# LiuZhu-CV/PAIF

Hardware: AMD Instinct MI355X
Metric: fused image-pairs/sec at 480x640 bs=8 per GPU (fusion-net forward) (higher is better)
Workload: dtype f16 (IEEE fp16 maps and conv weights, one fp16 MFMA per product, f32 accumulate; stems, guided filter and the last map fp32)

## Files before the change

paif_amd/csrc/conv_dma.hip:

```cpp
#include <stdint.h>
#include <stdlib.h>

#include <type_traits>

#include "conv_dma.h"
#include "paif_common.h"

namespace paif_conv_dma {
namespace {

typedef float f32x16 __attribute__((ext_vector_type(16)));
typedef unsigned u32x4 __attribute__((ext_vector_type(4)));
constexpr int TW = 32, TH = 8;
#ifndef CD_PF
#define CD_PF 4
#endif
#ifndef CD_ST_AUX
#define CD_ST_AUX 2
#endif
#ifndef CD_EXP
#define CD_EXP 0
#endif
constexpr int PARK_WAVE = 2 * 32 * 32 * 4;
template <int DIL>
struct Geo {
  static constexpr int TWH = TW + 2 * DIL, THH = TH + 2 * DIL;
  static constexpr int NPIX = TWH * THH;
  static constexpr int DPW = (NPIX * 4 + 255) / 256;
  static constexpr int SLOT = 4 * DPW * 1024;
  static constexpr int PF = DIL == 1 ? CD_PF : 3;
  static constexpr int NSLOT = PF + 1;
  static constexpr int ROWB = TWH * 64;
  static constexpr int PARK_OFF = NSLOT * SLOT;
  static constexpr int LDS_BYTES = PARK_OFF + 4 * PARK_WAVE;
  static_assert(LDS_BYTES <= 160 * 1024, "ring + transposition buffers exceed LDS");
  static_assert(4 * DPW * 64 >= NPIX * 4, "DMA instructions do not cover the halo tile");
  static __device__ __forceinline__ int base_row(int w) { return DIL == 1 ? 2 * w : (w >> 1) * 4 + (w & 1); }
};
constexpr unsigned RSRC_W3 = 0x00020000u;
constexpr unsigned OOB = 0x80000000u;
constexpr int NSTORE = 4;
constexpr int VMCAP = 63;

#define CD_VMWAIT(n) asm volatile("s_waitcnt vmcnt(%0)" ::"n"((n) > VMCAP ? VMCAP : (n)) : "memory")
#define CD_RD128(dst, addr, off) asm volatile("ds_read_b128 %0, %1 offset:%2" : "=v"(dst) : "v"(addr), "n"(off) : "memory")
#define CD_WR32(addr, val, off) asm volatile("ds_write_b32 %0, %1 offset:%2" ::"v"(addr), "v"(val), "n"(off) : "memory")

__device__ __forceinline__ void dma16(__amdgpu_buffer_rsrc_t rsrc, unsigned voff, unsigned lds_off) {
  __builtin_amdgcn_raw_ptr_buffer_load_lds(rsrc, (__attribute__((address_space(3))) void*)(uintptr_t)lds_off, 16, voff, 0, 0, 0);
}

template <int NSRC, int NRES, int PF, int DPW>
struct Sched {
  static constexpr int RL = 4 * NRES;
  static constexpr int smod(int x) { return ((x % NSRC) + NSRC) % NSRC; }
  static constexpr int R_STAGE = smod(1 - PF);
  static constexpr int D = (R_STAGE + PF - 1 - NSRC) / NSRC;
  static constexpr int U = D + (R_STAGE == 0 ? 2 : 1);
  static_assert(PF >= 2 && D >= 0 && U <= 4, "prefetch distance out of the range the tile loop lists");
  static constexpr int n1 = DPW * (PF - 1);
};

template <int NSRC, int NRES, int F, bool CP = false, int DIL = 1, int IA = 0>
__global__ __launch_bounds__(256, 1) void conv3x3_h16_dma(Args a, int ntiles, int tilesX, int tilesY) {
  typedef Geo<DIL> G;
  constexpr int TWH = G::TWH, NPIX = G::NPIX, DPW = G::DPW, SLOT = G::SLOT, PF = G::PF, NSLOT = G::NSLOT, ROWB = G::ROWB, PARK_OFF = G::PARK_OFF;
  typedef Sched<NSRC, NRES, PF, DPW> SC;
  constexpr int U = SC::U, D = SC::D;
  __shared__ __attribute__((aligned(16))) unsigned char smem[G::LDS_BYTES];
  asm volatile("" ::"v"((unsigned)(uintptr_t)(__attribute__((address_space(3))) unsigned char*)smem) : "memory");

  const int tid = threadIdx.x, l = tid & 63;
  const int w = __builtin_amdgcn_readfirstlane(tid >> 6);
  const int p = l & 31, hh = l >> 5;
  const int wb = G::base_row(w);

  const int xcd = blockIdx.x & 7, wg = blockIdx.x >> 3, nwg = gridDim.x >> 3;
  const int tpx = (ntiles + 7) >> 3;
  const int t_beg = xcd * tpx, t_end = min(ntiles, t_beg + tpx);
  const int cnt = t_beg + wg < t_end ? (t_end - t_beg - wg + nwg - 1) / nwg : 0;
  if (cnt == 0) return;
  const int H = a.H, W = a.W;
  auto pack_tile = [&](int k) -> unsigned {
    const int pos = wg + min(k, cnt - 1) * nwg;
    int t = a.reverse ? t_end - 1 - pos : t_beg + pos;
    const int tx = t % tilesX;
    t /= tilesX;
    const int ty = t % tilesY;
    return ((unsigned)(t / tilesY) << 22) | ((unsigned)ty << 11) | (unsigned)tx;
  };
  const unsigned tab0 = pack_tile(l), tab1 = pack_tile(l + 64);
  auto tile_of = [&](int k, int& b, int& y0, int& x0) -> bool {
    const bool ok = k >= 0 && k < cnt;
    const int kk = ok ? k : 0;
    const unsigned lo = __builtin_amdgcn_readlane(tab0, kk & 63), hi = __builtin_amdgcn_readlane(tab1, kk & 63);
    const unsigned pk = kk < 64 ? lo : hi;
    b = pk >> 22; y0 = ((pk >> 11) & 2047) * TH; x0 = (pk & 2047) * TW;
    return ok;
  };

  const int map_bytes = a.B * H * W * 64;
  __amdgpu_buffer_rsrc_t rs_src[NSRC];
#pragma unroll
  for (int s = 0; s < NSRC; ++s) rs_src[s] = __builtin_amdgcn_make_buffer_rsrc(const_cast<void*>(a.src[s]), 0, map_bytes, RSRC_W3);
  __amdgpu_buffer_rsrc_t rs_res[NRES > 0 ? NRES : 1];
#pragma unroll
  for (int r = 0; r < NRES; ++r) rs_res[r] = __builtin_amdgcn_make_buffer_rsrc(const_cast<void*>(a.res[r]), 0, map_bytes, RSRC_W3);
  const int opitch = a.cout * 2;
  const __amdgpu_buffer_rsrc_t rs_out = __builtin_amdgcn_make_buffer_rsrc(a.out, 0, a.B * H * W * opitch, RSRC_W3);
  const __amdgpu_buffer_rsrc_t rs_null = __builtin_amdgcn_make_buffer_rsrc(a.out, 0, 0, RSRC_W3);
  const __amdgpu_buffer_rsrc_t rs_cp = __builtin_amdgcn_make_buffer_rsrc(CP ? (void*)a.cpool : a.out, 0, CP ? a.B * H * W * 16 - 8 : 0, RSRC_W3);

  u32x4 bw[NSRC][9][2];
  {
    const __amdgpu_buffer_rsrc_t rs_w = __builtin_amdgcn_make_buffer_rsrc(const_cast<void*>(a.wpk), 0, NSRC * 9 * 2 * 2 * 1024, RSRC_W3);
#pragma unroll
    for (int s = 0; s < NSRC; ++s)
#pragma unroll
      for (int tap = 0; tap < 9; ++tap)
#pragma unroll
        for (int ks = 0; ks < 2; ++ks)
          bw[s][tap][ks] = __builtin_amdgcn_raw_buffer_load_b128(rs_w, (unsigned)l * 16u, (((s * 9 + tap) * 2 + ks) * 2) * 1024, 0);
  }
  float esc[8], esh[8];
#pragma unroll
  for (int j = 0; j < 8; ++j) {
    const int c = 8 * (l & 3) + j;
    esc[j] = ((a.scale && c < a.cout) ? a.scale[c] : 1.f) * a.alpha;
    esh[j] = ((a.shift && c < a.cout) ? a.shift[c] : 0.f) * a.alpha;
  }
  const float e_slope = a.act == 1 ? *a.prelu : (a.act == 2 ? 0.f : 1.f);

  int d_rel[DPW];
  int d_rc[DPW];
#pragma unroll
  for (int i = 0; i < DPW; ++i) {
    const int n = (w * DPW + i) * 64 + l;
    const int pi = n >> 2;
    const int r = pi / TWH, c = pi - r * TWH;
    d_rel[i] = (r * W + c) * 64 + (((n & 3) ^ ((c >> 2) & 3)) * 16);
    d_rc[i] = pi < NPIX ? (r | (c << 8)) : -1;
  }
  unsigned d_voff[DPW];
  auto target = [&](int k) {
    int b, y0, x0;
    const bool ok = tile_of(k, b, y0, x0);
    const int org = ((b * H + y0 - DIL) * W + x0 - DIL) * 64;
#pragma unroll
    for (int i = 0; i < DPW; ++i) {
      const int gy = y0 - DIL + (d_rc[i] & 0xff), gx = x0 - DIL + (d_rc[i] >> 8);
      const bool in = !(CD_EXP & 4) && ok && d_rc[i] >= 0 && (unsigned)gy < (unsigned)H && (unsigned)gx < (unsigned)W;
      d_voff[i] = in ? (unsigned)(org + d_rel[i]) : OOB;
    }
  };
  unsigned a_rd[3][2];
#pragma unroll
  for (int dx = 0; dx < 3; ++dx)
#pragma unroll
    for (int ks = 0; ks < 2; ++ks) {
      const int c = p + dx * DIL;
      a_rd[dx][ks] = (unsigned)(wb * ROWB + c * 64 + (((2 * ks + hh) ^ ((c >> 2) & 3)) * 16));
    }
  const unsigned a_pw = PARK_OFF + w * PARK_WAVE + (4 * hh * 32 + p) * 4;
  const unsigned a_pr = PARK_OFF + w * PARK_WAVE + (l >> 2) * 128 + (l & 3) * 32;
  const unsigned e_lane = (unsigned)l * 16u;
  const unsigned o_lane = 8 * (l & 3) < a.cout ? (unsigned)((l >> 2) * opitch + (l & 3) * 16) : OOB;

  u32x4 rr[U][NRES > 0 ? NRES : 1][4];
  auto issue_res = [&](auto settag, int k) {
    constexpr int SET = decltype(settag)::value;
    int b, y0, x0;
    const bool ok = tile_of(k, b, y0, x0);
#pragma unroll
    for (int it = 0; it < 4; ++it) {
      const int y = y0 + wb + (it >> 1) * DIL, x = x0 + (it & 1) * 16 + (l >> 2);
      const bool in = ok && y < H && x < W;
      const unsigned soff = (unsigned)(((b * H + y) * W + x0 + (it & 1) * 16) * 64);
#pragma unroll
      for (int r = 0; r < NRES; ++r) rr[SET][r][it] = __builtin_amdgcn_raw_buffer_load_b128(rs_res[r], in ? e_lane : OOB, soff, 0);
    }
  };

  auto relu_frag = [](u32x4& f) {
    typedef short s16x8 __attribute__((ext_vector_type(8)));
    const s16x8 z = {0, 0, 0, 0, 0, 0, 0, 0};
    f = __builtin_bit_cast(u32x4, __builtin_elementwise_max(__builtin_bit_cast(s16x8, f), z));
  };
  f32x16 acc[2];
  u32x4 t[4][2];
#pragma unroll
  for (int it = 0; it < 4; ++it) t[it][0] = t[it][1] = u32x4{0, 0, 0, 0};
  float ev[8];
  float pmx = 0.f, psm = 0.f;
  int cur = NSLOT - PF;

  auto epi = [&](auto mtag, auto settag, bool pok, int pb, int py0, int px0) {
    constexpr int M = decltype(mtag)::value, SETP = decltype(settag)::value;
    constexpr int it = M / 9, j = M % 9;
    if constexpr (j < 8) {
      const unsigned raw = j < 4 ? t[it][0][j & 3] : t[it][1][j & 3];
      float v = __builtin_fmaf(__uint_as_float(raw), esc[j], esh[j]);
      v = __builtin_fmaf(e_slope, fminf(v, 0.f), fmaxf(v, 0.f));
#pragma unroll
      for (int r = 0; r < NRES; ++r) {
        const unsigned u = rr[SETP][r][it][j >> 1];
        if constexpr (F == 2) v += (float)__builtin_bit_cast(paif::f16x2_t, u)[j & 1];
        else v += __uint_as_float((j & 1) ? (u & 0xffff0000u) : (u << 16));
      }
      ev[j] = v;
      if constexpr (CP) {
        pmx = j == 0 ? v : fmaxf(pmx, v);
        psm = j == 0 ? v : psm + v;
      }
    } else {
      const uint2 o0 = paif::f32_to_h4<F>(make_float4(ev[0], ev[1], ev[2], ev[3]));
      const uint2 o1 = paif::f32_to_h4<F>(make_float4(ev[4], ev[5], ev[6], ev[7]));
      const int y = py0 + wb + (it >> 1) * DIL, x = px0 + (it & 1) * 16 + (l >> 2);
      const unsigned soff = (unsigned)(((pb * H + y) * W + px0 + (it & 1) * 16) * opitch);
      u32x4 od = {o0.x, o0.y, o1.x, o1.y};
      __builtin_amdgcn_raw_buffer_store_b128(od, rs_out, (!(CD_EXP & 1) && pok && y < H && x < W) ? o_lane : OOB, soff, CD_ST_AUX);
      asm volatile("s_nop 2" : "+v"(od));
      if constexpr (CP) {
        float mx = pmx, sm = psm;
        mx = fmaxf(mx, paif::dpp_f<0xB1>(mx)); sm += paif::dpp_f<0xB1>(sm);
        mx = fmaxf(mx, paif::dpp_f<0x4E>(mx)); sm += paif::dpp_f<0x4E>(sm);
        typedef float f32x2v __attribute__((ext_vector_type(2)));
        const f32x2v pv = {mx, sm * (1.0f / 32.0f)};
        const unsigned poff = (unsigned)(((pb * H + y) * W + px0 + (it & 1) * 16) * 16);
        __builtin_amdgcn_raw_buffer_store_b64(__builtin_bit_cast(unsigned __attribute__((ext_vector_type(2))), pv), rs_cp,
                                              (pok && y < H && x < W && (l & 3) == 0) ? (unsigned)((l >> 2) * 16) : OOB, poff, 0);
      }
    }
  };

  auto stage = [&](auto ktag, auto stag, auto virt, int k) {
    constexpr int K = decltype(ktag)::value, S = decltype(stag)::value;
    constexpr bool VIRT = decltype(virt)::value;
    constexpr int SETP = (K + U - 1) % U;
    const unsigned sb = (unsigned)cur * SLOT;
    const int fill = cur == 0 ? NSLOT - 1 : cur - 1;
    u32x4 A[2][4];
    unsigned ad[3][2];
    if constexpr (!VIRT) {
      CD_VMWAIT(SC::n1);
      asm volatile("s_barrier" ::: "memory");
#pragma unroll
      for (int dx = 0; dx < 3; ++dx)
#pragma unroll
        for (int ks = 0; ks < 2; ++ks) ad[dx][ks] = a_rd[dx][ks] + sb;
      if constexpr (S == 0) {
#pragma unroll
        for (int it = 0; it < 4; ++it) {
          CD_RD128(t[it][0], a_pr, it * 2048);
          CD_RD128(t[it][1], a_pr, it * 2048 + 16);
        }
      }
#pragma unroll
      for (int r = 0; r < 4; ++r) CD_RD128(A[0][r], ad[0][0], r * DIL * ROWB);
    }
    if constexpr (NRES > 0 && S == SC::R_STAGE) issue_res(std::integral_constant<int, (K + D) % U>{}, k + D);
    asm volatile("" ::: "memory");
    if constexpr ((S + PF) % NSRC == 0) target(k + (S + PF) / NSRC);
#pragma unroll
    for (int i = 0; i < DPW; ++i) dma16(rs_src[(S + PF) % NSRC], d_voff[i], (unsigned)(fill * SLOT + (w * DPW + i) * 1024));
    if constexpr (VIRT) {
      if constexpr (S == 0) {
#pragma unroll
        for (int it = 0; it < NSTORE; ++it) __builtin_amdgcn_raw_buffer_store_b128(u32x4{0, 0, 0, 0}, rs_null, 0, 0, 0);
      }
    } else {
      int pb = 0, py0 = 0, px0 = 0;
      bool pok = false;
      if constexpr (S == 0) pok = tile_of(k - 1, pb, py0, px0);
      auto mma = [&](auto gitag, auto dytag, auto jtag) {
        constexpr int gi = decltype(gitag)::value, dy = decltype(dytag)::value, j = decltype(jtag)::value;
        constexpr int ks = gi / 3, dx = gi % 3;
        if constexpr (!((CD_EXP & 2) && (dy > 0 || j > 0))) {
          const u32x4 av = A[gi & 1][j + dy], bv = bw[S][dy * 3 + dx][ks];
          if constexpr (S == 0 && gi == 0 && dy == 0) {
            const f32x16 z = {0.f, 0.f, 0.f, 0.f, 0.f, 0.f, 0.f, 0.f, 0.f, 0.f, 0.f, 0.f, 0.f, 0.f, 0.f, 0.f};
            acc[j] = paif::mfma16<F>(av, bv, z);
          } else {
            acc[j] = paif::mfma16<F>(av, bv, acc[j]);
          }
        }
        if constexpr (S == 0) epi(std::integral_constant<int, gi * 6 + dy * 2 + j>{}, std::integral_constant<int, SETP>{}, pok, pb, py0, px0);
        if constexpr (IA == 2) {
          constexpr int call = dy * 2 + j;
          if constexpr (call == 0) relu_frag(A[gi & 1][1]);
          if constexpr (call == 2) relu_frag(A[gi & 1][2]);
          if constexpr (call == 4) relu_frag(A[gi & 1][3]);
        }
        __builtin_amdgcn_sched_barrier(0);
      };
      auto group = [&](auto gitag) {
        constexpr int gi = decltype(gitag)::value;
        if constexpr (gi + 1 < 6) {
          constexpr int ks1 = (gi + 1) / 3, dx1 = (gi + 1) % 3;
#pragma unroll
          for (int r = 0; r < 4; ++r) CD_RD128(A[(gi + 1) & 1][r], ad[dx1][ks1], r * DIL * ROWB);
        }
        if constexpr (S == 0 && gi == 0) {
          asm volatile("s_waitcnt lgkmcnt(4)"
                       : "+v"(A[0][0]), "+v"(A[0][1]), "+v"(A[0][2]), "+v"(A[0][3]), "+v"(t[0][0]), "+v"(t[0][1]), "+v"(t[1][0]), "+v"(t[1][1]),
                         "+v"(t[2][0]), "+v"(t[2][1]), "+v"(t[3][0]), "+v"(t[3][1])::"memory");
        } else if constexpr (gi + 1 < 6) {
          asm volatile("s_waitcnt lgkmcnt(4)" : "+v"(A[gi & 1][0]), "+v"(A[gi & 1][1]), "+v"(A[gi & 1][2]), "+v"(A[gi & 1][3])::"memory");
        } else {
          asm volatile("s_waitcnt lgkmcnt(0)" : "+v"(A[gi & 1][0]), "+v"(A[gi & 1][1]), "+v"(A[gi & 1][2]), "+v"(A[gi & 1][3])::"memory");
        }
        if constexpr (IA == 2) relu_frag(A[gi & 1][0]);
        __builtin_amdgcn_sched_barrier(0);
        typedef std::integral_constant<int, 0> I0;
        typedef std::integral_constant<int, 1> I1;
        typedef std::integral_constant<int, 2> I2;
        mma(gitag, I0{}, I0{}); mma(gitag, I0{}, I1{});
        mma(gitag, I1{}, I0{}); mma(gitag, I1{}, I1{});
        mma(gitag, I2{}, I0{}); mma(gitag, I2{}, I1{});
      };
      group(std::integral_constant<int, 0>{});
      group(std::integral_constant<int, 1>{});
      group(std::integral_constant<int, 2>{});
      group(std::integral_constant<int, 3>{});
      group(std::integral_constant<int, 4>{});
      group(std::integral_constant<int, 5>{});
      if constexpr (S == NSRC - 1) {
        asm volatile("s_nop 15\n\ts_nop 7" ::: "memory");
#pragma unroll
        for (int j = 0; j < 2; ++j)
#pragma unroll
          for (int r = 0; r < 16; ++r) {
            const float v = acc[j][r];
            CD_WR32(a_pw, v, (j * 32 + (r & 3) + 8 * (r >> 2)) * 128);
          }
      }
    }
    cur = cur == NSLOT - 1 ? 0 : cur + 1;
  };
  auto drain = [&](auto ktag, int k) {
    constexpr int K = decltype(ktag)::value;
#pragma unroll
    for (int it = 0; it < 4; ++it) {
      CD_RD128(t[it][0], a_pr, it * 2048);
      CD_RD128(t[it][1], a_pr, it * 2048 + 16);
    }
    asm volatile("s_waitcnt lgkmcnt(0)"
                 : "+v"(t[0][0]), "+v"(t[0][1]), "+v"(t[1][0]), "+v"(t[1][1]), "+v"(t[2][0]), "+v"(t[2][1]), "+v"(t[3][0]), "+v"(t[3][1])::"memory");
    int pb, py0, px0;
    const bool pok = tile_of(k, pb, py0, px0);
#define CD_M(m) epi(std::integral_constant<int, m>{}, std::integral_constant<int, K>{}, pok, pb, py0, px0);
    CD_M(0) CD_M(1) CD_M(2) CD_M(3) CD_M(4) CD_M(5) CD_M(6) CD_M(7) CD_M(8) CD_M(9) CD_M(10) CD_M(11)
    CD_M(12) CD_M(13) CD_M(14) CD_M(15) CD_M(16) CD_M(17) CD_M(18) CD_M(19) CD_M(20) CD_M(21) CD_M(22) CD_M(23)
    CD_M(24) CD_M(25) CD_M(26) CD_M(27) CD_M(28) CD_M(29) CD_M(30) CD_M(31) CD_M(32) CD_M(33) CD_M(34) CD_M(35)
#undef CD_M
  };

  auto vstage = [&](auto jtag) {
    constexpr int J = decltype(jtag)::value;
    constexpr int T = (J - (NSRC - 1)) / NSRC;
    constexpr int S = J - T * NSRC;
    constexpr int K = ((T % U) + U) % U;
    stage(std::integral_constant<int, K>{}, std::integral_constant<int, S>{}, std::true_type{}, T);
  };
  static_assert(PF >= 1 && PF <= 4, "the prologue lists up to 4 virtual stages");
  if constexpr (PF >= 4) vstage(std::integral_constant<int, -4>{});
  if constexpr (PF >= 3) vstage(std::integral_constant<int, -3>{});
  if constexpr (PF >= 2) vstage(std::integral_constant<int, -2>{});
  vstage(std::integral_constant<int, -1>{});

  auto tile_step = [&](auto ktag, int k) {
    stage(ktag, std::integral_constant<int, 0>{}, std::false_type{}, k);
    if constexpr (NSRC > 1) stage(ktag, std::integral_constant<int, 1>{}, std::false_type{}, k);
    if constexpr (NSRC > 2) stage(ktag, std::integral_constant<int, 2>{}, std::false_type{}, k);
  };
  for (int k = 0;; k += U) {
    tile_step(std::integral_constant<int, 0>{}, k);
    if (k + 1 >= cnt) { drain(std::integral_constant<int, 0>{}, k); break; }
    if constexpr (U > 1) {
      tile_step(std::integral_constant<int, 1 % U>{}, k + 1);
      if (k + 2 >= cnt) { drain(std::integral_constant<int, 1 % U>{}, k + 1); break; }
    }
    if constexpr (U > 2) {
      tile_step(std::integral_constant<int, 2 % U>{}, k + 2);
      if (k + 3 >= cnt) { drain(std::integral_constant<int, 2 % U>{}, k + 2); break; }
    }
    if constexpr (U > 3) {
      tile_step(std::integral_constant<int, 3 % U>{}, k + 3);
      if (k + 4 >= cnt) { drain(std::integral_constant<int, 3 % U>{}, k + 3); break; }
    }
  }
  CD_VMWAIT(0);
}

namespace k7 {
constexpr int P = 3;
constexpr int TWH = TW + 2 * P, THH = TH + 2 * P;
constexpr int NPIX = TWH * THH;
constexpr int DPW = 9;
constexpr int SLOT = 4 * DPW * 1024;
constexpr int NSLOT = 2;
constexpr int ROWB = TWH * 64;
constexpr int WB_OFF = NSLOT * SLOT;
constexpr int WB_BYTES = 49 * 1024;
constexpr int PARK_OFF = WB_OFF + WB_BYTES;
constexpr int LDS_BYTES = PARK_OFF + 4 * PARK_WAVE;
static_assert(LDS_BYTES <= 160 * 1024, "7x7: ring + weights + transposition buffers exceed LDS");
static_assert(4 * DPW * 64 >= NPIX * 4, "7x7: DMA instructions do not cover the halo tile");
}

#define CD_WR128(addr, val, off) asm volatile("ds_write_b128 %0, %1 offset:%2" ::"v"(addr), "v"(val), "n"(off) : "memory")

template <int F>
__global__ __launch_bounds__(256, 1) void conv7x7_h16_dma(Args a, int ntiles, int tilesX, int tilesY) {
  constexpr int P = k7::P, TWH = k7::TWH, NPIX = k7::NPIX, DPW = k7::DPW, SLOT = k7::SLOT, ROWB = k7::ROWB, WB_OFF = k7::WB_OFF,
                PARK_OFF = k7::PARK_OFF;
  __shared__ __attribute__((aligned(16))) unsigned char smem[k7::LDS_BYTES];
  asm volatile("" ::"v"((unsigned)(uintptr_t)(__attribute__((address_space(3))) unsigned char*)smem) : "memory");

  const int tid = threadIdx.x, l = tid & 63;
  const int w = __builtin_amdgcn_readfirstlane(tid >> 6);
  const int p = l & 31, hh = l >> 5;
  const int xcd = blockIdx.x & 7, wg = blockIdx.x >> 3, nwg = gridDim.x >> 3;
  const int tpx = (ntiles + 7) >> 3;
  const int t_beg = xcd * tpx, t_end = min(ntiles, t_beg + tpx);
  const int cnt = t_beg + wg < t_end ? (t_end - t_beg - wg + nwg - 1) / nwg : 0;
  if (cnt == 0) return;
  const int H = a.H, W = a.W;
  auto pack_tile = [&](int k) -> unsigned {
    const int pos = wg + min(k, cnt - 1) * nwg;
    int t = a.reverse ? t_end - 1 - pos : t_beg + pos;
    const int tx = t % tilesX;
    t /= tilesX;
    const int ty = t % tilesY;
    return ((unsigned)(t / tilesY) << 22) | ((unsigned)ty << 11) | (unsigned)tx;
  };
  const unsigned tab0 = pack_tile(l), tab1 = pack_tile(l + 64);
  auto tile_of = [&](int k, int& b, int& y0, int& x0) -> bool {
    const bool ok = k >= 0 && k < cnt;
    const int kk = ok ? k : 0;
    const unsigned lo = __builtin_amdgcn_readlane(tab0, kk & 63), hi = __builtin_amdgcn_readlane(tab1, kk & 63);
    const unsigned pk = kk < 64 ? lo : hi;
    b = pk >> 22; y0 = ((pk >> 11) & 2047) * TH; x0 = (pk & 2047) * TW;
    return ok;
  };
  const int map_bytes = a.B * H * W * 64;
  const __amdgpu_buffer_rsrc_t rs_src = __builtin_amdgcn_make_buffer_rsrc(const_cast<void*>(a.src[0]), 0, map_bytes, RSRC_W3);
  const __amdgpu_buffer_rsrc_t rs_out = __builtin_amdgcn_make_buffer_rsrc(a.out, 0, map_bytes, RSRC_W3);
  const __amdgpu_buffer_rsrc_t rs_w = __builtin_amdgcn_make_buffer_rsrc(const_cast<void*>(a.wpk), 0, 49 * 2 * 2 * 1024, RSRC_W3);

  u32x4 bw0[49];
#pragma unroll
  for (int tap = 0; tap < 49; ++tap) bw0[tap] = __builtin_amdgcn_raw_buffer_load_b128(rs_w, (unsigned)l * 16u, ((tap * 2 + 0) * 2) * 1024, 0);
#pragma unroll 1
  for (int i = tid; i < 49 * 64; i += 256) {
    const int tap = i >> 6, ln = i & 63;
    const u32x4 v = __builtin_amdgcn_raw_buffer_load_b128(rs_w, (unsigned)ln * 16u, ((tap * 2 + 1) * 2) * 1024, 0);
    const unsigned dst = WB_OFF + (unsigned)i * 16u;
    CD_WR128(dst, v, 0);
  }
  float esc[8], esh[8];
#pragma unroll
  for (int j = 0; j < 8; ++j) {
    const int c = 8 * (l & 3) + j;
    esc[j] = (a.scale ? a.scale[c] : 1.f) * a.alpha;
    esh[j] = (a.shift ? a.shift[c] : 0.f) * a.alpha;
  }
  const float e_slope = a.act == 1 ? *a.prelu : (a.act == 2 ? 0.f : 1.f);

  int d_rel[DPW], d_rc[DPW];
#pragma unroll
  for (int i = 0; i < DPW; ++i) {
    const int n = (w * DPW + i) * 64 + l;
    const int pi = n >> 2;
    const int r = pi / TWH, c = pi - r * TWH;
    d_rel[i] = (r * W + c) * 64 + (((n & 3) ^ ((c >> 2) & 3)) * 16);
    d_rc[i] = pi < NPIX ? (r | (c << 8)) : -1;
  }
  unsigned d_voff[DPW];
  auto target = [&](int k) {
    int b, y0, x0;
    const bool ok = tile_of(k, b, y0, x0);
    const int org = ((b * H + y0 - P) * W + x0 - P) * 64;
#pragma unroll
    for (int i = 0; i < DPW; ++i) {
      const int gy = y0 - P + (d_rc[i] & 0xff), gx = x0 - P + (d_rc[i] >> 8);
      const bool in = ok && d_rc[i] >= 0 && (unsigned)gy < (unsigned)H && (unsigned)gx < (unsigned)W;
      d_voff[i] = in ? (unsigned)(org + d_rel[i]) : OOB;
    }
  };
  unsigned a_rd[7][2];
#pragma unroll
  for (int dx = 0; dx < 7; ++dx)
#pragma unroll
    for (int ks = 0; ks < 2; ++ks) {
      const int c = p + dx;
      a_rd[dx][ks] = (unsigned)(2 * w * ROWB + c * 64 + (((2 * ks + hh) ^ ((c >> 2) & 3)) * 16));
    }
  const unsigned a_wb = WB_OFF + (unsigned)l * 16u;
  const unsigned a_pw = PARK_OFF + w * PARK_WAVE + (4 * hh * 32 + p) * 4;
  const unsigned a_pr = PARK_OFF + w * PARK_WAVE + (l >> 2) * 128 + (l & 3) * 32;
  const unsigned e_lane = (unsigned)l * 16u;

  f32x16 acc[2];
  u32x4 t[4][2];
#pragma unroll
  for (int it = 0; it < 4; ++it) t[it][0] = t[it][1] = u32x4{0, 0, 0, 0};
  float ev[8];
  auto epi = [&](auto mtag, bool pok, int pb, int py0, int px0) {
    constexpr int M = decltype(mtag)::value;
    constexpr int it = M / 9, j = M % 9;
    if constexpr (j < 8) {
      const unsigned raw = j < 4 ? t[it][0][j & 3] : t[it][1][j & 3];
      float v = __builtin_fmaf(__uint_as_float(raw), esc[j], esh[j]);
      ev[j] = __builtin_fmaf(e_slope, fminf(v, 0.f), fmaxf(v, 0.f));
    } else {
      const uint2 o0 = paif::f32_to_h4<F>(make_float4(ev[0], ev[1], ev[2], ev[3]));
      const uint2 o1 = paif::f32_to_h4<F>(make_float4(ev[4], ev[5], ev[6], ev[7]));
      const int y = py0 + 2 * w + (it >> 1), x = px0 + (it & 1) * 16 + (l >> 2);
      const unsigned soff = (unsigned)(((pb * H + y) * W + px0 + (it & 1) * 16) * 64);
      u32x4 od = {o0.x, o0.y, o1.x, o1.y};
      __builtin_amdgcn_raw_buffer_store_b128(od, rs_out, (pok && y < H && x < W) ? e_lane : OOB, soff, CD_ST_AUX);
      asm volatile("s_nop 2" : "+v"(od));
    }
  };

  asm volatile("s_waitcnt lgkmcnt(0)" ::: "memory");
  target(0);
#pragma unroll
  for (int i = 0; i < DPW; ++i) dma16(rs_src, d_voff[i], (unsigned)((w * DPW + i) * 1024));
  int cur = 0;
  for (int k = 0; k < cnt; ++k) {
    const unsigned sb = (unsigned)cur * SLOT;
    CD_VMWAIT(0);
    asm volatile("s_barrier" ::: "memory");
    unsigned ad[7][2];
#pragma unroll
    for (int dx = 0; dx < 7; ++dx)
#pragma unroll
      for (int ks = 0; ks < 2; ++ks) ad[dx][ks] = a_rd[dx][ks] + sb;
    u32x4 A[2][8], BL[7];
#pragma unroll
    for (int it = 0; it < 4; ++it) {
      CD_RD128(t[it][0], a_pr, it * 2048);
      CD_RD128(t[it][1], a_pr, it * 2048 + 16);
    }
#pragma unroll
    for (int r = 0; r < 8; ++r) CD_RD128(A[0][r], ad[0][0], r * ROWB);
    target(k + 1);
#pragma unroll
    for (int i = 0; i < DPW; ++i) dma16(rs_src, d_voff[i], (unsigned)((cur ^ 1) * SLOT + (w * DPW + i) * 1024));
    int pb, py0, px0;
    const bool pok = tile_of(k - 1, pb, py0, px0);
    auto mma = [&](auto gitag, auto dytag, auto jtag) {
      constexpr int gi = decltype(gitag)::value, dy = decltype(dytag)::value, j = decltype(jtag)::value;
      constexpr int dx = gi >> 1, ks = gi & 1;
      const u32x4 av = A[gi & 1][j + dy];
      const u32x4 bv = ks == 0 ? bw0[dy * 7 + dx] : BL[dy];
      if constexpr (gi == 0 && dy == 0) {
        const f32x16 z = {0.f, 0.f, 0.f, 0.f, 0.f, 0.f, 0.f, 0.f, 0.f, 0.f, 0.f, 0.f, 0.f, 0.f, 0.f, 0.f};
        acc[j] = paif::mfma16<F>(av, bv, z);
      } else {
        acc[j] = paif::mfma16<F>(av, bv, acc[j]);
      }
      constexpr int m = gi * 14 + dy * 2 + j;
      if constexpr (m < 36) epi(std::integral_constant<int, m>{}, pok, pb, py0, px0);
      __builtin_amdgcn_sched_barrier(0);
    };
    auto group = [&](auto gitag) {
      constexpr int gi = decltype(gitag)::value;
      if constexpr (gi + 1 < 14) {
        constexpr int dx1 = (gi + 1) >> 1, ks1 = (gi + 1) & 1;
#pragma unroll
        for (int r = 0; r < 8; ++r) CD_RD128(A[(gi + 1) & 1][r], ad[dx1][ks1], r * ROWB);
        if constexpr (ks1 == 1) {
#pragma unroll
          for (int dy = 0; dy < 7; ++dy) CD_RD128(BL[dy], a_wb, (dy * 7 + dx1) * 1024);
        }
      }
      if constexpr (gi == 0) {
        asm volatile("s_waitcnt lgkmcnt(15)"
                     : "+v"(A[0][0]), "+v"(A[0][1]), "+v"(A[0][2]), "+v"(A[0][3]), "+v"(A[0][4]), "+v"(A[0][5]), "+v"(A[0][6]), "+v"(A[0][7]),
                       "+v"(t[0][0]), "+v"(t[0][1]), "+v"(t[1][0]), "+v"(t[1][1]), "+v"(t[2][0]), "+v"(t[2][1]), "+v"(t[3][0])::"memory");
        asm volatile("" : "+v"(t[3][1])::"memory");
      } else if constexpr (gi + 1 >= 14) {
        asm volatile("s_waitcnt lgkmcnt(0)"
                     : "+v"(A[1][0]), "+v"(A[1][1]), "+v"(A[1][2]), "+v"(A[1][3]), "+v"(A[1][4]), "+v"(A[1][5]), "+v"(A[1][6]), "+v"(A[1][7]),
                       "+v"(BL[0]), "+v"(BL[1]), "+v"(BL[2]), "+v"(BL[3]), "+v"(BL[4]), "+v"(BL[5]), "+v"(BL[6])::"memory");
      } else if constexpr ((gi & 1) == 1) {
        asm volatile("s_waitcnt lgkmcnt(8)"
                     : "+v"(A[1][0]), "+v"(A[1][1]), "+v"(A[1][2]), "+v"(A[1][3]), "+v"(A[1][4]), "+v"(A[1][5]), "+v"(A[1][6]), "+v"(A[1][7]),
                       "+v"(BL[0]), "+v"(BL[1]), "+v"(BL[2]), "+v"(BL[3]), "+v"(BL[4]), "+v"(BL[5]), "+v"(BL[6])::"memory");
      } else {
        asm volatile("s_waitcnt lgkmcnt(15)"
                     : "+v"(A[0][0]), "+v"(A[0][1]), "+v"(A[0][2]), "+v"(A[0][3]), "+v"(A[0][4]), "+v"(A[0][5]), "+v"(A[0][6]), "+v"(A[0][7])::"memory");
      }
      __builtin_amdgcn_sched_barrier(0);
      typedef std::integral_constant<int, 0> J0;
      typedef std::integral_constant<int, 1> J1;
#define CD_DY(d) mma(gitag, std::integral_constant<int, d>{}, J0{}); mma(gitag, std::integral_constant<int, d>{}, J1{});
      CD_DY(0) CD_DY(1) CD_DY(2) CD_DY(3) CD_DY(4) CD_DY(5) CD_DY(6)
#undef CD_DY
    };
#define CD_G(g) group(std::integral_constant<int, g>{});
    CD_G(0) CD_G(1) CD_G(2) CD_G(3) CD_G(4) CD_G(5) CD_G(6) CD_G(7) CD_G(8) CD_G(9) CD_G(10) CD_G(11) CD_G(12) CD_G(13)
#undef CD_G
    asm volatile("s_nop 15\n\ts_nop 7" ::: "memory");
#pragma unroll
    for (int j = 0; j < 2; ++j)
#pragma unroll
      for (int r = 0; r < 16; ++r) {
        const float v = acc[j][r];
        CD_WR32(a_pw, v, (j * 32 + (r & 3) + 8 * (r >> 2)) * 128);
      }
    cur ^= 1;
  }
  {
#pragma unroll
    for (int it = 0; it < 4; ++it) {
      CD_RD128(t[it][0], a_pr, it * 2048);
      CD_RD128(t[it][1], a_pr, it * 2048 + 16);
    }
    asm volatile("s_waitcnt lgkmcnt(0)"
                 : "+v"(t[0][0]), "+v"(t[0][1]), "+v"(t[1][0]), "+v"(t[1][1]), "+v"(t[2][0]), "+v"(t[2][1]), "+v"(t[3][0]), "+v"(t[3][1])::"memory");
    int pb, py0, px0;
    const bool pok = tile_of(cnt - 1, pb, py0, px0);
#define CD_M(m) epi(std::integral_constant<int, m>{}, pok, pb, py0, px0);
    CD_M(0) CD_M(1) CD_M(2) CD_M(3) CD_M(4) CD_M(5) CD_M(6) CD_M(7) CD_M(8) CD_M(9) CD_M(10) CD_M(11)
    CD_M(12) CD_M(13) CD_M(14) CD_M(15) CD_M(16) CD_M(17) CD_M(18) CD_M(19) CD_M(20) CD_M(21) CD_M(22) CD_M(23)
    CD_M(24) CD_M(25) CD_M(26) CD_M(27) CD_M(28) CD_M(29) CD_M(30) CD_M(31) CD_M(32) CD_M(33) CD_M(34) CD_M(35)
#undef CD_M
  }
  CD_VMWAIT(0);
}

int launch_7(const Args& a, hipStream_t st) {
  const int tilesX = (a.W + TW - 1) / TW, tilesY = (a.H + TH - 1) / TH;
  if (a.f16) hipLaunchKernelGGL(conv7x7_h16_dma<2>, dim3(256), dim3(256), 0, st, a, a.B * tilesX * tilesY, tilesX, tilesY);
  else hipLaunchKernelGGL(conv7x7_h16_dma<1>, dim3(256), dim3(256), 0, st, a, a.B * tilesX * tilesY, tilesX, tilesY);
  hipError_t e = hipGetLastError();
  if (e != hipSuccess) {
    paif::set_error("conv2d(bf16 dma 7x7): launch failed: %s", hipGetErrorString(e));
    return (int)e;
  }
  return 0;
}

template <int NSRC, int NRES>
int launch_n(const Args& a, hipStream_t st) {
  const int tilesX = (a.W + TW - 1) / TW, tilesY = (a.H + TH - 1) / TH;
  if (a.cpool) {
    if constexpr (NSRC == 3 && (NRES == 1 || NRES == 3)) {
      if (a.f16) hipLaunchKernelGGL((conv3x3_h16_dma<NSRC, NRES, 2, true>), dim3(256), dim3(256), 0, st, a, a.B * tilesX * tilesY, tilesX, tilesY);
      else hipLaunchKernelGGL((conv3x3_h16_dma<NSRC, NRES, 1, true>), dim3(256), dim3(256), 0, st, a, a.B * tilesX * tilesY, tilesX, tilesY);
    } else {
      paif::set_error("conv2d(dma): the fused ChannelPool is built for 3 sources with 1 or 3 residual maps");
      return PAIF_ENOSUP;
    }
  } else if (a.f16) hipLaunchKernelGGL((conv3x3_h16_dma<NSRC, NRES, 2>), dim3(256), dim3(256), 0, st, a, a.B * tilesX * tilesY, tilesX, tilesY);
  else hipLaunchKernelGGL((conv3x3_h16_dma<NSRC, NRES, 1>), dim3(256), dim3(256), 0, st, a, a.B * tilesX * tilesY, tilesX, tilesY);
  hipError_t e = hipGetLastError();
  if (e != hipSuccess) {
    paif::set_error("conv2d(h16 dma): launch failed: %s", hipGetErrorString(e));
    return (int)e;
  }
  return 0;
}

template <int NRES, bool CP>
int launch_d2(const Args& a, hipStream_t st) {
  const int tilesX = (a.W + TW - 1) / TW, tilesY = (a.H + TH - 1) / TH;
  if (a.f16) hipLaunchKernelGGL((conv3x3_h16_dma<1, NRES, 2, CP, 2, 2>), dim3(256), dim3(256), 0, st, a, a.B * tilesX * tilesY, tilesX, tilesY);
  else hipLaunchKernelGGL((conv3x3_h16_dma<1, NRES, 1, CP, 2, 2>), dim3(256), dim3(256), 0, st, a, a.B * tilesX * tilesY, tilesX, tilesY);
  hipError_t e = hipGetLastError();
  if (e != hipSuccess) {
    paif::set_error("conv2d(h16 dma, dilation 2): launch failed: %s", hipGetErrorString(e));
    return (int)e;
  }
  return 0;
}

}

bool eligible(int nsrc, int nres, int B, int H, int W, float alpha) {
  static const bool on = [] {
    const char* e = getenv("PAIF_CONV_DMA");
    return !(e && e[0] == '0');
  }();
  if (!on || nsrc < 1 || nsrc > 3 || nres < 0 || nres > 3 || !(alpha > 0.f)) return false;
  if (nsrc == 1 && nres > 1) return false;
  const long long tiles = (long long)B * ((H + TH - 1) / TH) * ((W + TW - 1) / TW);
  return tiles >= 1024 && tiles <= 128 * 256 && B < 1024 && H < 2048 * TH && W < 2048 * TW && (long long)B * H * W * 64 < (1ll << 31);
}

bool eligible_d2(int nsrc, int nres, int B, int H, int W, float alpha) {
  static const bool on = [] {
    const char* e = getenv("PAIF_CONV_DMA_D2");
    return !(e && e[0] == '0');
  }();
  return on && nsrc == 1 && (nres == 1 || nres == 3) && eligible(1, 1, B, H, W, alpha);
}

bool eligible16(int nsrc, int nres, int B, int H, int W, float alpha) { return nsrc == 1 && nres == 0 && eligible(1, 0, B, H, W, alpha); }
bool eligible7(int nsrc, int nres, int B, int H, int W, float alpha) { return nsrc == 1 && nres == 0 && eligible(1, 0, B, H, W, alpha); }

bool can_cpool(int nsrc, int nres, int kh, int cout, int dil) {
  return kh == 3 && cout == 32 && ((dil == 1 && nsrc == 3 && (nres == 1 || nres == 3)) || (dil == 2 && nsrc == 1 && (nres == 1 || nres == 3)));
}

int launch(const Args& a, hipStream_t st) {
  if (a.cpool && !can_cpool(a.nsrc, a.nres, a.kh, a.cout, a.dil)) {
    paif::set_error("conv2d(dma): no fused ChannelPool for this form");
    return PAIF_ENOSUP;
  }
  if (a.kh == 7) return launch_7(a, st);
  if (a.dil == 2) {
    if (a.nsrc == 1 && a.in_relu && a.nres == 1) return a.cpool ? launch_d2<1, true>(a, st) : launch_d2<1, false>(a, st);
    if (a.nsrc == 1 && a.in_relu && a.nres == 3) return a.cpool ? launch_d2<3, true>(a, st) : launch_d2<3, false>(a, st);
    paif::set_error("conv2d(h16 dma): dilation 2 is built for one source behind an input ReLU with 1 or 3 residual maps");
    return PAIF_ENOSUP;
  }
  if (a.in_relu) {
    paif::set_error("conv2d(h16 dma): the input ReLU is built for the dilation-2 form");
    return PAIF_ENOSUP;
  }
  switch (a.nsrc * 10 + a.nres) {
    case 10: return launch_n<1, 0>(a, st);
    case 11: return launch_n<1, 1>(a, st);
    case 20: return launch_n<2, 0>(a, st);
    case 21: return launch_n<2, 1>(a, st);
    case 22: return launch_n<2, 2>(a, st);
    case 23: return launch_n<2, 3>(a, st);
    case 30: return launch_n<3, 0>(a, st);
    case 31: return launch_n<3, 1>(a, st);
    case 32: return launch_n<3, 2>(a, st);
    case 33: return launch_n<3, 3>(a, st);
    default: break;
  }
  paif::set_error("conv2d(bf16 dma): %d sources / %d residual maps not built", a.nsrc, a.nres);
  return PAIF_ENOSUP;
}

}
```

Before: 2481.

## Add 8-wave 32x16 tile variant of the single-source 3x3 DMA conv

Adds an 8-wave (512-thread) build of the 3x3 DMA conv kernel for the single-source, no-residual case. Each workgroup covers a 32x16 tile, which amortises halo traffic and puts more waves on each CU. To fit LDS, the prefetch depth drops to 2 and the transposition park area is halved, so accumulators are parked and read back one row at a time. A host-side heuristic, overridable through PAIF_CONV_DMA_NW, selects this path when the tile count falls in a set range. The cost is a shallower prefetch ring and a serialised park/readback.

```diff
diff --git a/paif_amd/csrc/conv_dma.hip b/paif_amd/csrc/conv_dma.hip
--- a/paif_amd/csrc/conv_dma.hip
+++ b/paif_amd/csrc/conv_dma.hip
@@ -1,5 +1,6 @@
 #include <stdint.h>
 #include <stdlib.h>
+#include <string.h>
 
 #include <type_traits>
 
@@ -22,19 +23,22 @@
 #define CD_EXP 0
 #endif
 constexpr int PARK_WAVE = 2 * 32 * 32 * 4;
-template <int DIL>
+template <int DIL, int NW = 4>
 struct Geo {
+  static constexpr int TH = 2 * NW;
   static constexpr int TWH = TW + 2 * DIL, THH = TH + 2 * DIL;
   static constexpr int NPIX = TWH * THH;
-  static constexpr int DPW = (NPIX * 4 + 255) / 256;
-  static constexpr int SLOT = 4 * DPW * 1024;
-  static constexpr int PF = DIL == 1 ? CD_PF : 3;
+  static constexpr int DPW = (NPIX * 4 + NW * 64 - 1) / (NW * 64);
+  static constexpr int SLOT = NW * DPW * 1024;
+  static constexpr int PF = NW == 8 ? 2 : DIL == 1 ? CD_PF : 3;
   static constexpr int NSLOT = PF + 1;
   static constexpr int ROWB = TWH * 64;
+  static constexpr int PARK_W = NW == 8 ? PARK_WAVE / 2 : PARK_WAVE;
   static constexpr int PARK_OFF = NSLOT * SLOT;
-  static constexpr int LDS_BYTES = PARK_OFF + 4 * PARK_WAVE;
+  static constexpr int LDS_BYTES = PARK_OFF + NW * PARK_W;
+  static_assert(NW == 4 || (NW == 8 && DIL == 1), "the 8-wave build is dilation 1 only");
   static_assert(LDS_BYTES <= 160 * 1024, "ring + transposition buffers exceed LDS");
-  static_assert(4 * DPW * 64 >= NPIX * 4, "DMA instructions do not cover the halo tile");
+  static_assert(NW * DPW * 64 >= NPIX * 4, "DMA instructions do not cover the halo tile");
   static __device__ __forceinline__ int base_row(int w) { return DIL == 1 ? 2 * w : (w >> 1) * 4 + (w & 1); }
 };
 constexpr unsigned RSRC_W3 = 0x00020000u;
@@ -61,10 +65,11 @@
   static constexpr int n1 = DPW * (PF - 1);
 };
 
-template <int NSRC, int NRES, int F, bool CP = false, int DIL = 1, int IA = 0>
-__global__ __launch_bounds__(256, 1) void conv3x3_h16_dma(Args a, int ntiles, int tilesX, int tilesY) {
-  typedef Geo<DIL> G;
+template <int NSRC, int NRES, int F, bool CP = false, int DIL = 1, int IA = 0, int NW = 4>
+__global__ __launch_bounds__(64 * NW, 1) void conv3x3_h16_dma(Args a, int ntiles, int tilesX, int tilesY) {
+  typedef Geo<DIL, NW> G;
   constexpr int TWH = G::TWH, NPIX = G::NPIX, DPW = G::DPW, SLOT = G::SLOT, PF = G::PF, NSLOT = G::NSLOT, ROWB = G::ROWB, PARK_OFF = G::PARK_OFF;
+  constexpr int TH = G::TH, PARK_W = G::PARK_W;
   typedef Sched<NSRC, NRES, PF, DPW> SC;
   constexpr int U = SC::U, D = SC::D;
   __shared__ __attribute__((aligned(16))) unsigned char smem[G::LDS_BYTES];
@@ -161,8 +166,8 @@
       const int c = p + dx * DIL;
       a_rd[dx][ks] = (unsigned)(wb * ROWB + c * 64 + (((2 * ks + hh) ^ ((c >> 2) & 3)) * 16));
     }
-  const unsigned a_pw = PARK_OFF + w * PARK_WAVE + (4 * hh * 32 + p) * 4;
-  const unsigned a_pr = PARK_OFF + w * PARK_WAVE + (l >> 2) * 128 + (l & 3) * 32;
+  const unsigned a_pw = PARK_OFF + w * PARK_W + (4 * hh * 32 + p) * 4;
+  const unsigned a_pr = PARK_OFF + w * PARK_W + (l >> 2) * 128 + (l & 3) * 32;
   const unsigned e_lane = (unsigned)l * 16u;
   const unsigned o_lane = 8 * (l & 3) < a.cout ? (unsigned)((l >> 2) * opitch + (l & 3) * 16) : OOB;
 
@@ -181,15 +186,50 @@
     }
   };
 
+  f32x16 acc[2];
+  u32x4 t[4][2];
+#pragma unroll
+  for (int it = 0; it < 4; ++it) t[it][0] = t[it][1] = u32x4{0, 0, 0, 0};
+  auto park_row = [&](int j, int off) {
+#pragma unroll
+    for (int r = 0; r < 16; ++r) {
+      const float v = acc[j][r];
+      CD_WR32(a_pw, v, off + ((r & 3) + 8 * (r >> 2)) * 128);
+    }
+  };
+  auto read_back = [&]() {
+    if constexpr (NW == 8) {
+      asm volatile("s_nop 15\n\ts_nop 7" ::: "memory");
+      park_row(0, 0);
+#pragma unroll
+      for (int it = 0; it < 2; ++it) {
+        CD_RD128(t[it][0], a_pr, it * 2048);
+        CD_RD128(t[it][1], a_pr, it * 2048 + 16);
+      }
+      park_row(1, 0);
+#pragma unroll
+      for (int it = 2; it < 4; ++it) {
+        CD_RD128(t[it][0], a_pr, (it & 1) * 2048);
+        CD_RD128(t[it][1], a_pr, (it & 1) * 2048 + 16);
+      }
+    } else {
+#pragma unroll
+      for (int it = 0; it < 4; ++it) {
+        CD_RD128(t[it][0], a_pr, it * 2048);
+        CD_RD128(t[it][1], a_pr, it * 2048 + 16);
+      }
+    }
+  };
+
   auto relu_frag = [](u32x4& f) {
     typedef short s16x8 __attribute__((ext_vector_type(8)));
     const s16x8 z = {0, 0, 0, 0, 0, 0, 0, 0};
     f = __builtin_bit_cast(u32x4, __builtin_elementwise_max(__builtin_bit_cast(s16x8, f), z));
   };
-  f32x16 acc[2];
-  u32x4 t[4][2];
-#pragma unroll
-  for (int it = 0; it < 4; ++it) t[it][0] = t[it][1] = u32x4{0, 0, 0, 0};
+#pragma unroll
+  for (int j = 0; j < 2; ++j)
+#pragma unroll
+    for (int r = 0; r < 16; ++r) acc[j][r] = 0.f;
   float ev[8];
   float pmx = 0.f, psm = 0.f;
   int cur = NSLOT - PF;
@@ -248,13 +288,7 @@
       for (int dx = 0; dx < 3; ++dx)
 #pragma unroll
         for (int ks = 0; ks < 2; ++ks) ad[dx][ks] = a_rd[dx][ks] + sb;
-      if constexpr (S == 0) {
-#pragma unroll
-        for (int it = 0; it < 4; ++it) {
-          CD_RD128(t[it][0], a_pr, it * 2048);
-          CD_RD128(t[it][1], a_pr, it * 2048 + 16);
-        }
-      }
+      if constexpr (S == 0) read_back();
 #pragma unroll
       for (int r = 0; r < 4; ++r) CD_RD128(A[0][r], ad[0][0], r * DIL * ROWB);
     }
@@ -324,26 +358,17 @@
       group(std::integral_constant<int, 3>{});
       group(std::integral_constant<int, 4>{});
       group(std::integral_constant<int, 5>{});
-      if constexpr (S == NSRC - 1) {
+      if constexpr (S == NSRC - 1 && NW == 4) {
         asm volatile("s_nop 15\n\ts_nop 7" ::: "memory");
-#pragma unroll
-        for (int j = 0; j < 2; ++j)
-#pragma unroll
-          for (int r = 0; r < 16; ++r) {
-            const float v = acc[j][r];
-            CD_WR32(a_pw, v, (j * 32 + (r & 3) + 8 * (r >> 2)) * 128);
-          }
+        park_row(0, 0);
+        park_row(1, 32 * 128);
       }
     }
     cur = cur == NSLOT - 1 ? 0 : cur + 1;
   };
   auto drain = [&](auto ktag, int k) {
     constexpr int K = decltype(ktag)::value;
-#pragma unroll
-    for (int it = 0; it < 4; ++it) {
-      CD_RD128(t[it][0], a_pr, it * 2048);
-      CD_RD128(t[it][1], a_pr, it * 2048 + 16);
-    }
+    read_back();
     asm volatile("s_waitcnt lgkmcnt(0)"
                  : "+v"(t[0][0]), "+v"(t[0][1]), "+v"(t[1][0]), "+v"(t[1][1]), "+v"(t[2][0]), "+v"(t[2][1]), "+v"(t[3][0]), "+v"(t[3][1])::"memory");
     int pb, py0, px0;
@@ -646,18 +671,45 @@
 }
 
 template <int NSRC, int NRES>
+constexpr bool kHasNW8 = NSRC == 1 && NRES == 0;
+
+int nw_of(const Args& a, bool has8, int& tilesY) {
+  const char* e = getenv("PAIF_CONV_DMA_NW");
+  if (e && strcmp(e, "4") && strcmp(e, "8")) return -1;
+  const int tilesX = (a.W + TW - 1) / TW, ty8 = (a.H + 15) / 16;
+  const long long tiles8 = (long long)a.B * ty8 * tilesX;
+  if (has8 && !(e && !strcmp(e, "4")) && tiles8 >= 1024 && tiles8 <= 128 * 256) {
+    tilesY = ty8;
+    return 8;
+  }
+  tilesY = (a.H + TH - 1) / TH;
+  return 4;
+}
+
+template <int NSRC, int NRES>
 int launch_n(const Args& a, hipStream_t st) {
-  const int tilesX = (a.W + TW - 1) / TW, tilesY = (a.H + TH - 1) / TH;
+  int tilesY;
+  const int nw = nw_of(a, kHasNW8<NSRC, NRES> && !a.cpool, tilesY);
+  if (nw < 0) {
+    paif::set_error("PAIF_CONV_DMA_NW must be 4 or 8 (got '%s')", getenv("PAIF_CONV_DMA_NW"));
+    return PAIF_EINVAL;
+  }
+  const int tilesX = (a.W + TW - 1) / TW, ntiles = a.B * tilesX * tilesY;
   if (a.cpool) {
     if constexpr (NSRC == 3 && (NRES == 1 || NRES == 3)) {
-      if (a.f16) hipLaunchKernelGGL((conv3x3_h16_dma<NSRC, NRES, 2, true>), dim3(256), dim3(256), 0, st, a, a.B * tilesX * tilesY, tilesX, tilesY);
-      else hipLaunchKernelGGL((conv3x3_h16_dma<NSRC, NRES, 1, true>), dim3(256), dim3(256), 0, st, a, a.B * tilesX * tilesY, tilesX, tilesY);
+      if (a.f16) hipLaunchKernelGGL((conv3x3_h16_dma<NSRC, NRES, 2, true>), dim3(256), dim3(256), 0, st, a, ntiles, tilesX, tilesY);
+      else hipLaunchKernelGGL((conv3x3_h16_dma<NSRC, NRES, 1, true>), dim3(256), dim3(256), 0, st, a, ntiles, tilesX, tilesY);
     } else {
       paif::set_error("conv2d(dma): the fused ChannelPool is built for 3 sources with 1 or 3 residual maps");
       return PAIF_ENOSUP;
     }
-  } else if (a.f16) hipLaunchKernelGGL((conv3x3_h16_dma<NSRC, NRES, 2>), dim3(256), dim3(256), 0, st, a, a.B * tilesX * tilesY, tilesX, tilesY);
-  else hipLaunchKernelGGL((conv3x3_h16_dma<NSRC, NRES, 1>), dim3(256), dim3(256), 0, st, a, a.B * tilesX * tilesY, tilesX, tilesY);
+  } else if (nw == 8) {
+    if constexpr (kHasNW8<NSRC, NRES>) {
+      if (a.f16) hipLaunchKernelGGL((conv3x3_h16_dma<NSRC, NRES, 2, false, 1, 0, 8>), dim3(256), dim3(512), 0, st, a, ntiles, tilesX, tilesY);
+      else hipLaunchKernelGGL((conv3x3_h16_dma<NSRC, NRES, 1, false, 1, 0, 8>), dim3(256), dim3(512), 0, st, a, ntiles, tilesX, tilesY);
+    }
+  } else if (a.f16) hipLaunchKernelGGL((conv3x3_h16_dma<NSRC, NRES, 2>), dim3(256), dim3(256), 0, st, a, ntiles, tilesX, tilesY);
+  else hipLaunchKernelGGL((conv3x3_h16_dma<NSRC, NRES, 1>), dim3(256), dim3(256), 0, st, a, ntiles, tilesX, tilesY);
   hipError_t e = hipGetLastError();
   if (e != hipSuccess) {
     paif::set_error("conv2d(h16 dma): launch failed: %s", hipGetErrorString(e));
```

Result: no change. 2483 (median of 6 runs) (+0.1%).
